# ps-auxw/CLI-P

Hardware: AMD Instinct MI355X
Metric: images/sec ViT-B/32 encode (higher is better)
Workload: dtype bf16

## Files before the change

### cli-p_amd/csrc/encode.hip

```cpp
#include "vit_kernels.hpp"

namespace clipmi {
namespace {

struct Ws {
    unsigned short* patches;
    float* x;
    unsigned short* h;
    unsigned short* big;
    unsigned short* pooled;
    int* rowidx;
    unsigned char* a8;
    float* a_scale;
    unsigned char* a_bs;
    unsigned char* x8;
    unsigned char* x8_bs;
    void* x3;
    float* ln_part;
    float* ln_leaf;
};

size_t carve(const clipmi_tower* t, int B, void* base, size_t cap, Ws* out) {
    Arena ar(base ? base : reinterpret_cast<void*>(256), cap);
    const size_t rows = (size_t)B * t->tokens;
    const int W = t->width;
    Ws w{};
    if (t->kind == 0) w.patches = ar.take<unsigned short>((size_t)B * (t->tokens - 1) * t->patch_k);
    w.x = ar.take<float>(rows * W);
    w.h = ar.take<unsigned short>(rows * W);
    w.big = ar.take<unsigned short>(rows * 4 * W);
    w.pooled = ar.take<unsigned short>((size_t)B * W);
    w.rowidx = ar.take<int>((size_t)B);
    if (t->weight_format == 1) {
        w.a8 = ar.take<unsigned char>(rows * 4 * W);
        w.a_scale = ar.take<float>(rows);
        w.a_bs = ar.take<unsigned char>((rows + 255) / 256 * 256 * (size_t)(4 * W / 32));
    }
    if (t->ln_fold && t->weight_format == 1) {
        w.x8 = ar.take<unsigned char>(rows * W);
        w.x8_bs = ar.take<unsigned char>((rows + 255) / 256 * 256 * (size_t)(W / 32));
        w.ln_part = ar.take<float>(rows * 2 * (W / 256));
    } else if (t->ln_fold) {
        w.x3 = ar.take<unsigned char>(rows * resid_row_bytes(W));
        w.ln_part = ar.take<float>(rows * 2 * (W / 256));
        if (rows <= (size_t)SKINNY_MAX_M) w.ln_leaf = ar.take<float>(rows * 2 * (W / 4));
    }
    if (out) *out = w;
    return ar.off + 256;
}

int check_tower(const clipmi_tower* t, int kind, const char* who) {
    if (!t) return set_err(CLIPMI_EINVAL, "%s: NULL tower", who);
    if (t->abi_version != CLIPMI_ABI_VERSION)
        return set_err(CLIPMI_EINVAL, "%s: tower ABI %d != %d", who, t->abi_version, CLIPMI_ABI_VERSION);
    if (t->kind != kind) return set_err(CLIPMI_EINVAL, "%s: tower kind %d", who, t->kind);
    if (t->width % 128 != 0 || t->heads * 64 != t->width || t->mlp != 4 * t->width || t->embed % 128 != 0 ||
        t->width > 1024 || t->layers < 1)
        return set_err(CLIPMI_EUNSUPPORTED,
                       "%s: width=%d heads=%d mlp=%d embed=%d (need width %% 128 == 0 <= 1024, head dim 64, embed %% 128 == 0)",
                       who, t->width, t->heads, t->mlp, t->embed);
    if (t->weight_format != 0 && t->weight_format != 1)
        return set_err(CLIPMI_EINVAL, "%s: weight_format %d", who, t->weight_format);
    if (t->weight_format == 1 && t->width % 256 != 0)
        return set_err(CLIPMI_EUNSUPPORTED, "%s: fp8 weights need width %% 256 == 0 (width %d)", who, t->width);
    if (t->ln_fold != 0 && (t->ln_fold != 1 || t->width % 256 != 0))
        return set_err(CLIPMI_EINVAL, "%s: ln_fold %d needs width %% 256 == 0 (width %d)", who, t->ln_fold, t->width);
#ifndef CLIPMI_DEV
    if (t->ln_fold != 0 && t->weight_format != 0)
        return set_err(CLIPMI_EUNSUPPORTED, "%s: folded LayerNorms on FP8 weights exist in the development library only", who);
#endif
    if (t->tokens > 80 && kind == 1)
        return set_err(CLIPMI_EUNSUPPORTED, "%s: %d tokens (causal attention covers <= 80)", who, t->tokens);
    return 0;
}

template <typename T>
const T* at(const void* blob, uint64_t off) {
    return reinterpret_cast<const T*>(static_cast<const char*>(blob) + off);
}

int run_layers(const clipmi_tower* t, const void* blob, const Ws& w, int B, int causal, hipStream_t st, GemmProbe* probe) {
    const int W = t->width, L = t->tokens, M = B * L;
    const bool fp8 = t->weight_format == 1;
    auto linear = [&](const unsigned short* A, int K, uint64_t w_off, uint64_t b_off, void* out, int N, int epi) -> int {
        GemmArgs g{};
        g.bias = at<float>(blob, b_off); g.out = out; g.M = M; g.N = N; g.K = K;
        g.A = A; g.W = at<unsigned short>(blob, w_off);
        return launch_gemm_algo(g, epi, 0, st, probe);
    };
#ifdef CLIPMI_DEV
    if (t->ln_fold && fp8) {
        auto lnfold8 = [&](uint64_t w_off, uint64_t s_off, uint64_t cb_off, uint64_t cs_off, void* out, unsigned char* out_bs, int N,
                           int epi) -> int {
            GemmArgs g{};
            g.A = reinterpret_cast<const unsigned short*>(w.x8); g.a_bscale = w.x8_bs;
            g.W = at<unsigned short>(blob, w_off); g.w_scale = at<float>(blob, s_off);
            g.bias = at<float>(blob, cb_off); g.colsum = at<float>(blob, cs_off); g.ln_part_in = w.ln_part;
            g.out = out; g.out_bscale = out_bs; g.M = M; g.N = N; g.K = W;
            return launch_gemm_fp8(g, epi, st);
        };
        auto resid8 = [&](const unsigned char* A8, int K, uint64_t w_off, uint64_t s_off, uint64_t b_off) -> int {
            GemmArgs g{};
            g.A = reinterpret_cast<const unsigned short*>(A8); g.a_bscale = w.a_bs;
            g.W = at<unsigned short>(blob, w_off); g.w_scale = at<float>(blob, s_off); g.bias = at<float>(blob, b_off);
            g.out = w.x; g.x8 = w.x8; g.x8_bs = w.x8_bs; g.ln_part = w.ln_part; g.M = M; g.N = W; g.K = K;
            return launch_gemm_fp8(g, EPI_BIAS_RESID_LN8, st);
        };
        unsigned char* const big8 = reinterpret_cast<unsigned char*>(w.big);
        static const bool fuse_off = dev_knob("CLIPMI_FP8_FUSE", 1) == 0;
        for (int l = 0; l < t->layers; ++l) {
            const uint64_t lb = t->off_layers + (uint64_t)l * t->layer_stride;
            if (int rc = lnfold8(lb + t->lo_qkv_w, lb + t->lo_qkv_s, lb + t->lo_qkv_cb, lb + t->lo_qkv_colsum, w.big, nullptr, 3 * W, EPI_LN_BIAS_BF16)) return rc;
            bool fused = false;
            if (int rc = launch_attention(w.big, w.h, B, L, t->heads, causal, 1, st, fuse_off ? nullptr : w.a8, w.a_bs, &fused)) return rc;
            if (!fused)
                if (int rc = launch_quantize_rows_fp8mx(w.h, w.a8, w.a_bs, M, W, st)) return rc;
            if (int rc = resid8(w.a8, W, lb + t->lo_out_w, lb + t->lo_out_s, lb + t->lo_out_b)) return rc;
            if (!fuse_off) {
                if (int rc = lnfold8(lb + t->lo_fc_w, lb + t->lo_fc_s, lb + t->lo_fc_cb, lb + t->lo_fc_colsum, big8, w.a_bs, 4 * W, EPI_LN_BIAS_QGELU_BF16)) return rc;
                if (int rc = resid8(big8, 4 * W, lb + t->lo_proj_w, lb + t->lo_proj_s, lb + t->lo_proj_b)) return rc;
            } else {
                if (int rc = lnfold8(lb + t->lo_fc_w, lb + t->lo_fc_s, lb + t->lo_fc_cb, lb + t->lo_fc_colsum, w.big, nullptr, 4 * W, EPI_LN_BIAS_QGELU_BF16)) return rc;
                if (int rc = launch_quantize_rows_fp8mx(w.big, w.a8, w.a_bs, M, 4 * W, st)) return rc;
                if (int rc = resid8(w.a8, 4 * W, lb + t->lo_proj_w, lb + t->lo_proj_s, lb + t->lo_proj_b)) return rc;
            }
        }
        return 0;
    }
#endif
    if (t->ln_fold) {
        auto lb_of = [&](int l) { return t->off_layers + (uint64_t)l * t->layer_stride; };
        const bool leaf_mode = w.ln_leaf != nullptr && gemm_resid_writes_leaves(M, W, W) && gemm_resid_writes_leaves(M, W, 4 * W);
        bool leaves = false;
        auto ln_linear = [&](uint64_t w_off, uint64_t cb_off, uint64_t cs_off, int N, int epi) -> int {
            GemmArgs g{};
            g.A = static_cast<const unsigned short*>(w.x3); g.lda_bytes = (unsigned)resid_row_bytes(W);
            g.W = at<unsigned short>(blob, w_off); g.bias = at<float>(blob, cb_off);
            g.colsum = at<float>(blob, cs_off); g.ln_part_in = w.ln_part;
            if (leaves) g.ln_leaf_in = w.ln_leaf;
            g.out = w.big; g.M = M; g.N = N; g.K = W;
            return launch_gemm_algo(g, epi, 0, st, probe);
        };
        auto resid_linear = [&](const unsigned short* A, int K, uint64_t w_off, uint64_t b_off) -> int {
            GemmArgs g{};
            g.A = A; g.W = at<unsigned short>(blob, w_off); g.bias = at<float>(blob, b_off);
            g.M = M; g.N = W; g.K = K;
            g.x3 = w.x3; g.ln_part = w.ln_part; g.tmp_f32 = w.x;
            if (leaf_mode) { g.ln_leaf = w.ln_leaf; leaves = true; }
            return launch_gemm_algo(g, EPI_BIAS_RESID_LN_F32, 0, st, probe);
        };
        for (int l = 0; l < t->layers; ++l) {
            const uint64_t lb = lb_of(l);
            if (int rc = ln_linear(lb + t->lo_qkv_w, lb + t->lo_qkv_cb, lb + t->lo_qkv_colsum, 3 * W, EPI_LN_BIAS_BF16)) return rc;
            hipEvent_t* aev = nullptr;
            if (probe && probe->mode == 2 && probe->n < GemmProbe::MAX) {
                const int pi = probe->begin(GemmProbe::EPI_ATTENTION, 2, st, 0);
                aev = &probe->ev[2 * pi];
            }
            if (int rc = launch_attention(w.big, w.h, B, L, t->heads, causal, 1, st, nullptr, nullptr, nullptr, aev)) return rc;
            if (int rc = resid_linear(w.h, W, lb + t->lo_out_w, lb + t->lo_out_b)) return rc;
            if (int rc = ln_linear(lb + t->lo_fc_w, lb + t->lo_fc_cb, lb + t->lo_fc_colsum, 4 * W, EPI_LN_BIAS_QGELU_BF16)) return rc;
            if (int rc = resid_linear(w.big, 4 * W, lb + t->lo_proj_w, lb + t->lo_proj_b)) return rc;
        }
        return 0;
    }
    if (fp8) {
        auto gemm8 = [&](const unsigned char* A8, const float* a_scale, const unsigned char* a_bs, int K, uint64_t w_off,
                         uint64_t s_off, uint64_t b_off, void* out, unsigned char* out_bs, int N, int epi) -> int {
            GemmArgs g{};
            g.bias = at<float>(blob, b_off); g.out = out; g.M = M; g.N = N; g.K = K;
            g.A = reinterpret_cast<const unsigned short*>(A8);
            g.W = at<unsigned short>(blob, w_off);
            g.a_scale = a_scale; g.a_bscale = a_bs; g.out_bscale = out_bs;
            g.w_scale = at<float>(blob, s_off);
            return launch_gemm_fp8(g, epi, st);
        };
        static const bool fuse_off = dev_knob("CLIPMI_FP8_FUSE", 1) == 0;
        const bool fc_mx = !fuse_off && gemm_fp8_emits_mx(M, 4 * W, W);
        unsigned char* const big8 = reinterpret_cast<unsigned char*>(w.big);
        for (int l = 0; l < t->layers; ++l) {
            const uint64_t lb = t->off_layers + (uint64_t)l * t->layer_stride;
            LnArgs ln{w.x, at<float>(blob, lb + t->lo_ln1_w), at<float>(blob, lb + t->lo_ln1_b), w.h, nullptr, 1, M, W, 1};
            ln.out8 = w.a8; ln.scale8 = w.a_scale;
            if (int rc = launch_layernorm(ln, st)) return rc;
            if (int rc = gemm8(w.a8, w.a_scale, nullptr, W, lb + t->lo_qkv_w, lb + t->lo_qkv_s, lb + t->lo_qkv_b, w.big, nullptr, 3 * W, EPI_BIAS_BF16)) return rc;
            bool fused = false;
            if (int rc = launch_attention(w.big, w.h, B, L, t->heads, causal, 1, st, fuse_off ? nullptr : w.a8, w.a_bs, &fused)) return rc;
            if (!fused)
                if (int rc = launch_quantize_rows_fp8mx(w.h, w.a8, w.a_bs, M, W, st)) return rc;
            if (int rc = gemm8(w.a8, nullptr, w.a_bs, W, lb + t->lo_out_w, lb + t->lo_out_s, lb + t->lo_out_b, w.x, nullptr, W, EPI_BIAS_RESID_F32)) return rc;
            ln.w = at<float>(blob, lb + t->lo_ln2_w); ln.b = at<float>(blob, lb + t->lo_ln2_b);
            if (int rc = launch_layernorm(ln, st)) return rc;
            const unsigned char* h8 = w.a8;
            if (fc_mx) {
                if (int rc = gemm8(w.a8, w.a_scale, nullptr, W, lb + t->lo_fc_w, lb + t->lo_fc_s, lb + t->lo_fc_b, big8, w.a_bs, 4 * W, EPI_BIAS_QGELU_BF16)) return rc;
                h8 = big8;
            } else {
                if (int rc = gemm8(w.a8, w.a_scale, nullptr, W, lb + t->lo_fc_w, lb + t->lo_fc_s, lb + t->lo_fc_b, w.big, nullptr, 4 * W, EPI_BIAS_QGELU_BF16)) return rc;
                if (int rc = launch_quantize_rows_fp8mx(w.big, w.a8, w.a_bs, M, 4 * W, st)) return rc;
            }
            if (int rc = gemm8(h8, nullptr, w.a_bs, 4 * W, lb + t->lo_proj_w, lb + t->lo_proj_s, lb + t->lo_proj_b, w.x, nullptr, W, EPI_BIAS_RESID_F32)) return rc;
        }
        return 0;
    }
    for (int l = 0; l < t->layers; ++l) {
        const uint64_t lb = t->off_layers + (uint64_t)l * t->layer_stride;
        LnArgs ln{w.x, at<float>(blob, lb + t->lo_ln1_w), at<float>(blob, lb + t->lo_ln1_b), w.h, nullptr, 1, M, W, 1};
        if (int rc = launch_layernorm(ln, st)) return rc;
        if (int rc = linear(w.h, W, lb + t->lo_qkv_w, lb + t->lo_qkv_b, w.big, 3 * W, EPI_BIAS_BF16)) return rc;
        if (int rc = launch_attention(w.big, w.h, B, L, t->heads, causal, 1, st)) return rc;
        if (int rc = linear(w.h, W, lb + t->lo_out_w, lb + t->lo_out_b, w.x, W, EPI_BIAS_RESID_F32)) return rc;
        ln.w = at<float>(blob, lb + t->lo_ln2_w); ln.b = at<float>(blob, lb + t->lo_ln2_b);
        if (int rc = launch_layernorm(ln, st)) return rc;
        if (int rc = linear(w.h, W, lb + t->lo_fc_w, lb + t->lo_fc_b, w.big, 4 * W, EPI_BIAS_QGELU_BF16)) return rc;
        if (int rc = linear(w.big, 4 * W, lb + t->lo_proj_w, lb + t->lo_proj_b, w.x, W, EPI_BIAS_RESID_F32)) return rc;
    }
    return 0;
}

int run_head(const clipmi_tower* t, const void* blob, const Ws& w, int B, const int* rowidx, long long row_step,
             float* out, int normalize, hipStream_t st) {
    const bool split = t->ln_fold && t->weight_format == 0;
    LnArgs ln{split ? nullptr : w.x, at<float>(blob, t->off_ln_post_w), at<float>(blob, t->off_ln_post_b), w.pooled, rowidx,
              row_step, B, t->width, 1};
    ln.x3 = w.x3;
    if (int rc = launch_layernorm(ln, st)) return rc;
    GemmArgs g{};
    g.A = w.pooled; g.W = at<unsigned short>(blob, t->off_out_proj); g.bias = nullptr; g.out = out;
    g.M = B; g.N = t->embed; g.K = t->width;
    if (int rc = launch_gemm_algo(g, EPI_F32, 0, st)) return rc;
    if (normalize) return clipmi_l2_normalize_rows(out, B, t->embed, st);
    return 0;
}

}
}

using namespace clipmi;

extern "C" size_t clipmi_encode_image_workspace_bytes(const clipmi_tower* t, int B) {
    if (check_tower(t, 0, "encode_image")) return 0;
    if (B < 1) { set_err(CLIPMI_EINVAL, "encode_image: B=%d", B); return 0; }
    return carve(t, B, nullptr, ~(size_t)0, nullptr);
}

static int encode_image_impl(const clipmi_tower* t, const void* blob_dev, const void* pixels_dev, int pix_dtype,
                             int B, float* out_dev, int normalize, void* ws_dev, size_t ws_bytes, void* stream, GemmProbe* probe) {
    if (int rc = check_tower(t, 0, "encode_image")) return rc;
    if (!blob_dev || !pixels_dev || !out_dev || !ws_dev) return set_err(CLIPMI_EINVAL, "encode_image: NULL pointer");
    if (B < 1) return set_err(CLIPMI_EINVAL, "encode_image: B=%d", B);
    if (pix_dtype != CLIPMI_F32 && pix_dtype != CLIPMI_BF16 && pix_dtype != CLIPMI_U8)
        return set_err(CLIPMI_EINVAL, "encode_image: pix_dtype %d", pix_dtype);
    const int grid = t->res / t->patch, np = grid * grid;
    if (np + 1 != t->tokens || t->patch_k % 64 != 0 || t->patch_k < 3 * t->patch * t->patch)
        return set_err(CLIPMI_EINVAL, "encode_image: inconsistent tower (res %d patch %d tokens %d patch_k %d)", t->res,
                       t->patch, t->tokens, t->patch_k);
    const size_t need = clipmi_encode_image_workspace_bytes(t, B);
    if (ws_bytes < need) return set_err(CLIPMI_EWORKSPACE, "encode_image: workspace %zu < %zu", ws_bytes, need);
    Ws w;
    carve(t, B, ws_dev, ws_bytes, &w);
    hipStream_t st = as_stream(stream);
    const int W = t->width, L = t->tokens;

    PatchArgs pa{pixels_dev, w.patches, pix_dtype, B, t->res, t->patch, grid, np, t->patch_k};
    if (int rc = launch_patchify(pa, st)) return rc;
    GemmArgs g{};
    g.A = w.patches; g.W = at<unsigned short>(blob_dev, t->off_patch_w); g.bias = nullptr; g.out = w.x;
    g.M = B * np; g.N = W; g.K = t->patch_k; g.pos = at<float>(blob_dev, t->off_pos); g.np = np; g.L = L;
    if (int rc = launch_gemm_algo(g, EPI_PATCH_F32, 0, st)) return rc;
    hipLaunchKernelGGL(cls_rows_kernel, dim3((unsigned)(((long long)B * W + 255) / 256)), dim3(256), 0, st, w.x,
                       at<float>(blob_dev, t->off_cls), at<float>(blob_dev, t->off_pos), B, L, W);
    CLIPMI_CHECK_LAUNCH("cls_rows_kernel");
    LnArgs ln{w.x, at<float>(blob_dev, t->off_ln_pre_w), at<float>(blob_dev, t->off_ln_pre_b), w.x, nullptr, 1, B * L, W, 0};
    const bool fold8 = t->ln_fold && t->weight_format == 1;
    if (t->ln_fold && !fold8) { ln.out_x3 = w.x3; ln.out_part = w.ln_part; }
    if (int rc = launch_layernorm(ln, st)) return rc;
#ifdef CLIPMI_DEV
    if (fold8)
        if (int rc = launch_rows_mx_stats(w.x, w.x8, w.x8_bs, w.ln_part, B * L, W, st)) return rc;
#endif
    if (int rc = run_layers(t, blob_dev, w, B, 0, st, probe)) return rc;
    return run_head(t, blob_dev, w, B, nullptr, L, out_dev, normalize, st);
}

extern "C" int clipmi_encode_image(const clipmi_tower* t, const void* blob_dev, const void* pixels_dev, int pix_dtype,
                                   int B, float* out_dev, int normalize, void* ws_dev, size_t ws_bytes, void* stream) {
    return encode_image_impl(t, blob_dev, pixels_dev, pix_dtype, B, out_dev, normalize, ws_dev, ws_bytes, stream, nullptr);
}

extern "C" size_t clipmi_encode_text_workspace_bytes(const clipmi_tower* t, int Q) {
    if (check_tower(t, 1, "encode_text")) return 0;
    if (Q < 1) { set_err(CLIPMI_EINVAL, "encode_text: Q=%d", Q); return 0; }
    return carve(t, Q, nullptr, ~(size_t)0, nullptr);
}

extern "C" int clipmi_encode_text(const clipmi_tower* t, const void* blob_dev, const int32_t* ids_dev, int Q,
                                  float* out_dev, int normalize, void* ws_dev, size_t ws_bytes, void* stream) {
    if (int rc = check_tower(t, 1, "encode_text")) return rc;
    if (!blob_dev || !ids_dev || !out_dev || !ws_dev) return set_err(CLIPMI_EINVAL, "encode_text: NULL pointer");
    if (Q < 1) return set_err(CLIPMI_EINVAL, "encode_text: Q=%d", Q);
    const size_t need = clipmi_encode_text_workspace_bytes(t, Q);
    if (ws_bytes < need) return set_err(CLIPMI_EWORKSPACE, "encode_text: workspace %zu < %zu", ws_bytes, need);
    Ws w;
    carve(t, Q, ws_dev, ws_bytes, &w);
    hipStream_t st = as_stream(stream);
    const int W = t->width, L = t->tokens;
    const long long n4 = (long long)Q * L * (W / 4);
    const bool fold8_ = t->ln_fold && t->weight_format == 1;
    if (t->ln_fold && !fold8_ && W % 256 == 0 && W <= 1024) {
        hipLaunchKernelGGL(text_embed_split_kernel, dim3((unsigned)((Q * L + 3) / 4 + 1)), dim3(256), 0, st, ids_dev,
                           at<float>(blob_dev, t->off_tok_emb), at<float>(blob_dev, t->off_pos), w.x3, w.ln_part, w.rowidx, Q, L, W,
                           t->vocab);
        CLIPMI_CHECK_LAUNCH("text_embed_split_kernel");
        if (int rc = run_layers(t, blob_dev, w, Q, 1, st, nullptr)) return rc;
        return run_head(t, blob_dev, w, Q, w.rowidx, 1, out_dev, normalize, st);
    }
    hipLaunchKernelGGL(text_embed_kernel, dim3((unsigned)((n4 + 255) / 256)), dim3(256), 0, st, w.x, ids_dev,
                       at<float>(blob_dev, t->off_tok_emb), at<float>(blob_dev, t->off_pos), Q, L, W, t->vocab);
    CLIPMI_CHECK_LAUNCH("text_embed_kernel");
    hipLaunchKernelGGL(eot_rows_kernel, dim3((Q + 63) / 64), dim3(64), 0, st, ids_dev, w.rowidx, Q, L);
    CLIPMI_CHECK_LAUNCH("eot_rows_kernel");
#ifdef CLIPMI_DEV
    if (t->ln_fold && t->weight_format == 1) {
        if (int rc = launch_rows_mx_stats(w.x, w.x8, w.x8_bs, w.ln_part, Q * L, W, st)) return rc;
    } else
#endif
    if (t->ln_fold) {
        if (int rc = launch_split_stats(w.x, false, w.x3, w.ln_part, Q * L, W, st)) return rc;
    }
    if (int rc = run_layers(t, blob_dev, w, Q, 1, st, nullptr)) return rc;
    return run_head(t, blob_dev, w, Q, w.rowidx, 1, out_dev, normalize, st);
}

static int encode_probe(const clipmi_tower* t, const void* blob_dev, const void* pixels_dev, int pix_dtype, int B, float* out_dev,
                        void* ws_dev, size_t ws_bytes, void* stream, int probe_epi, int reps, int nmodes, float* ms, int* launches,
                        int* kernel_kind, int* epi_ran) {
    if (!ms || reps < 1) return set_err(CLIPMI_EINVAL, "dbg_encode_image_probe_ms: bad arguments");
    const int k_filter = probe_epi >> 8;
    probe_epi &= 0xff;
    GemmProbe p;
    for (int i = 0; i < 2 * GemmProbe::MAX; ++i)
        if (hipEventCreate(&p.ev[i]) != hipSuccess) return set_err(CLIPMI_EHIP, "hipEventCreate");
    for (int i = 0; i < GemmProbe::MAX; ++i)
        if (hipEventCreate(&p.pre[i]) != hipSuccess) return set_err(CLIPMI_EHIP, "hipEventCreate");
    int rc = 0;
    for (int mode = 0; mode < nmodes && rc == 0; ++mode) {
        double total = 0.0;
        int count = 0;
        for (int r = 0; r < reps && rc == 0; ++r) {
            p.epi = probe_epi; p.n = 0; p.mode = mode;
            rc = encode_image_impl(t, blob_dev, pixels_dev, pix_dtype, B, out_dev, 1, ws_dev, ws_bytes, stream, &p);
            if (rc) break;
            if (hipStreamSynchronize(as_stream(stream)) != hipSuccess) { rc = set_err(CLIPMI_EHIP, "hipStreamSynchronize"); break; }
            for (int i = 0; i < p.n; ++i) {
                if (GemmProbe::base_of(p.epi_of[i]) != probe_epi || (k_filter && p.k_of[i] != k_filter)) continue;
                float v = 0.f;
                if (mode == 0) (void)hipEventElapsedTime(&v, p.ev[2 * i], p.ev[2 * i + 1]);
                else if (mode == 1) (void)hipEventElapsedTime(&v, p.pre[i], p.ev[2 * i + 1]);
                else {
                    if (i == 0 || p.kernel_of[i - 1] != 2 ||
                        (p.epi_of[i - 1] != EPI_BIAS_RESID_LN_F32 && p.epi_of[i - 1] != EPI_LN_BIAS_QGELU_BF16 &&
                         p.epi_of[i - 1] != GemmProbe::EPI_ATTENTION)) continue;
                    (void)hipEventElapsedTime(&v, p.ev[2 * (i - 1) + 1], p.ev[2 * i + 1]);
                }
                total += v;
                ++count;
                if (kernel_kind) *kernel_kind = p.kernel_of[i];
                if (epi_ran) *epi_ran = p.epi_of[i];
            }
        }
        if (rc == 0 && count == 0 && mode == 0) rc = set_err(CLIPMI_EINVAL, "dbg_encode_image_probe_ms: no launch matched epi %d", probe_epi);
        if (rc == 0) { ms[mode] = count ? (float)(total / count) : 0.f; if (launches && mode == 0) *launches = count; }
    }
    for (int i = 0; i < 2 * GemmProbe::MAX; ++i) (void)hipEventDestroy(p.ev[i]);
    for (int i = 0; i < GemmProbe::MAX; ++i) (void)hipEventDestroy(p.pre[i]);
    return rc;
}

extern "C" int clipmi_dbg_encode_image_probe_ms(const clipmi_tower* t, const void* blob_dev, const void* pixels_dev,
                                                int pix_dtype, int B, float* out_dev, void* ws_dev, size_t ws_bytes,
                                                void* stream, int probe_epi, int reps, float* kernel_ms, int* launches) {
    return encode_probe(t, blob_dev, pixels_dev, pix_dtype, B, out_dev, ws_dev, ws_bytes, stream, probe_epi, reps, 1, kernel_ms,
                        launches, nullptr, nullptr);
}

extern "C" int clipmi_dbg_encode_image_probe3_ms(const clipmi_tower* t, const void* blob_dev, const void* pixels_dev,
                                                 int pix_dtype, int B, float* out_dev, void* ws_dev, size_t ws_bytes,
                                                 void* stream, int probe_epi, int reps, float* ms3, int* launches,
                                                 int* kernel_kind, int* epi_ran) {
    return encode_probe(t, blob_dev, pixels_dev, pix_dtype, B, out_dev, ws_dev, ws_bytes, stream, probe_epi, reps, 3, ms3,
                        launches, kernel_kind, epi_ran);
}
```

### cli-p_amd/csrc/vit_kernels.hpp

```cpp
#pragma once
#include "gemm.hpp"

namespace clipmi {

struct PatchArgs {
    const void* pix;
    unsigned short* out;
    int dtype, B, R, P, grid, np, patch_k;
};

static __global__ void __launch_bounds__(256) patchify_kernel(PatchArgs a) {
    const long long total = (long long)a.B * a.np * (a.patch_k / 8);
    const long long i = (long long)blockIdx.x * 256 + threadIdx.x;
    if (i >= total) return;
    const int kc = a.patch_k / 8;
    const int k8 = (int)(i % kc);
    const long long bp = i / kc;
    const int p = (int)(bp % a.np);
    const int b = (int)(bp / a.np);
    const int PP = a.P * a.P;
    const float mean[3] = {0.48145466f, 0.4578275f, 0.40821073f};
    const float stdv[3] = {0.26862954f, 0.26130258f, 0.27577711f};
    float v[8];
    if ((a.P & 7) == 0 && (a.R & 7) == 0) {
        const int k = k8 * 8;
        if (k < 3 * PP) {
            const int c = k / PP, rem = k - c * PP;
            const int py = rem / a.P, px = rem - py * a.P;
            const int y = (p / a.grid) * a.P + py, xx = (p % a.grid) * a.P + px;
            const size_t src = (((size_t)b * 3 + c) * a.R + y) * a.R + xx;
            if (a.dtype == CLIPMI_F32) {
                const f32x4 lo = *reinterpret_cast<const f32x4*>(static_cast<const float*>(a.pix) + src);
                const f32x4 hi = *reinterpret_cast<const f32x4*>(static_cast<const float*>(a.pix) + src + 4);
                v[0] = lo.x; v[1] = lo.y; v[2] = lo.z; v[3] = lo.w; v[4] = hi.x; v[5] = hi.y; v[6] = hi.z; v[7] = hi.w;
            } else if (a.dtype == CLIPMI_BF16) {
                const uint4 raw = *reinterpret_cast<const uint4*>(static_cast<const unsigned short*>(a.pix) + src);
                const unsigned w[4] = {raw.x, raw.y, raw.z, raw.w};
#pragma unroll
                for (int j = 0; j < 4; ++j) {
                    v[2 * j] = __uint_as_float(w[j] << 16);
                    v[2 * j + 1] = __uint_as_float(w[j] & 0xffff0000u);
                }
            } else {
                const uint2 raw = *reinterpret_cast<const uint2*>(static_cast<const unsigned char*>(a.pix) + src);
                const float m = mean[c], s = stdv[c];
#pragma unroll
                for (int j = 0; j < 8; ++j) {
                    const unsigned byte = ((j < 4 ? raw.x : raw.y) >> (8 * (j & 3))) & 0xffu;
                    v[j] = ((float)byte / 255.0f - m) / s;
                }
            }
        } else {
#pragma unroll
            for (int j = 0; j < 8; ++j) v[j] = 0.f;
        }
    } else {
#pragma unroll
    for (int j = 0; j < 8; ++j) {
        const int k = k8 * 8 + j;
        float x = 0.f;
        if (k < 3 * PP) {
            const int c = k / PP, rem = k - c * PP;
            const int py = rem / a.P, px = rem - py * a.P;
            const int y = (p / a.grid) * a.P + py, xx = (p % a.grid) * a.P + px;
            const size_t src = (((size_t)b * 3 + c) * a.R + y) * a.R + xx;
            if (a.dtype == CLIPMI_F32) x = static_cast<const float*>(a.pix)[src];
            else if (a.dtype == CLIPMI_BF16) x = bf16_to_f32(static_cast<const unsigned short*>(a.pix)[src]);
            else x = ((float)static_cast<const unsigned char*>(a.pix)[src] / 255.0f - mean[c]) / stdv[c];
        }
        v[j] = x;
    }
    }
    uint4 o = make_uint4(pack_bf16x2(v[0], v[1]), pack_bf16x2(v[2], v[3]), pack_bf16x2(v[4], v[5]), pack_bf16x2(v[6], v[7]));
    *reinterpret_cast<uint4*>(a.out + ((size_t)bp * a.patch_k + k8 * 8)) = o;
}

static __global__ void __launch_bounds__(256) patchify_strip_u8_kernel(PatchArgs a) {
    extern __shared__ __attribute__((aligned(16))) char smem[];
    const int gy = blockIdx.x % a.grid;
    const int c = (blockIdx.x / a.grid) % 3;
    const int b = blockIdx.x / (3 * a.grid);
    const float mean[3] = {0.48145466f, 0.4578275f, 0.40821073f};
    const float stdv[3] = {0.26862954f, 0.26130258f, 0.27577711f};
    const float m = mean[c], sd = stdv[c];
    const unsigned char* src = static_cast<const unsigned char*>(a.pix) + (((size_t)b * 3 + c) * a.R + (size_t)gy * a.P) * a.R;
    unsigned short* lut = reinterpret_cast<unsigned short*>(smem + a.P * a.R);
    lut[threadIdx.x] = (unsigned short)(pack_bf16x2(((float)threadIdx.x / 255.0f - m) / sd, 0.f) & 0xffffu);
    const int nchunk = (a.P * a.R) >> 4;
    for (int j = threadIdx.x; j < nchunk; j += 256)
        *reinterpret_cast<uint4*>(smem + j * 16) = *reinterpret_cast<const uint4*>(src + (size_t)j * 16);
    __syncthreads();
    const int per_patch = (a.P * a.P) >> 3, per_row = a.P >> 3;
    for (int o = threadIdx.x; o < a.grid * per_patch; o += 256) {
        const int gx = o / per_patch, rem = o - gx * per_patch;
        const int y = rem / per_row, px = (rem - y * per_row) << 3;
        const uint2 raw = *reinterpret_cast<const uint2*>(smem + y * a.R + gx * a.P + px);
        unsigned w4[4];
#pragma unroll
        for (int k = 0; k < 4; ++k) {
            const unsigned word = k < 2 ? raw.x : raw.y;
            const unsigned b0 = (word >> (16 * (k & 1))) & 0xffu, b1 = (word >> (16 * (k & 1) + 8)) & 0xffu;
            w4[k] = (unsigned)lut[b0] | ((unsigned)lut[b1] << 16);
        }
        unsigned short* dst = a.out + ((size_t)b * a.np + gy * a.grid + gx) * a.patch_k + c * a.P * a.P + y * a.P + px;
        *reinterpret_cast<uint4*>(dst) = make_uint4(w4[0], w4[1], w4[2], w4[3]);
    }
}

static __global__ void __launch_bounds__(256) cls_rows_kernel(float* x, const float* cls, const float* pos, int B, int L, int W) {
    const long long i = (long long)blockIdx.x * 256 + threadIdx.x;
    if (i >= (long long)B * W) return;
    const int b = (int)(i / W), c = (int)(i - (long long)b * W);
    x[(size_t)b * L * W + c] = cls[c] + pos[c];
}

static __global__ void __launch_bounds__(256) text_embed_kernel(float* x, const int* ids, const float* tok, const float* pos,
                                                         int Q, int L, int W, int vocab) {
    const long long i = (long long)blockIdx.x * 256 + threadIdx.x;
    const int wc = W / 4;
    if (i >= (long long)Q * L * wc) return;
    const int c4 = (int)(i % wc);
    const long long row = i / wc;
    const int t = (int)(row % L);
    int id = ids[row];
    id = id < 0 ? 0 : (id >= vocab ? vocab - 1 : id);
    const f32x4 e = *reinterpret_cast<const f32x4*>(tok + (size_t)id * W + c4 * 4);
    const f32x4 p = *reinterpret_cast<const f32x4*>(pos + (size_t)t * W + c4 * 4);
    *reinterpret_cast<f32x4*>(x + (size_t)row * W + c4 * 4) = e + p;
}

static __global__ void eot_rows_kernel(const int* ids, int* rowidx, int Q, int L) {
    const int q = blockIdx.x * blockDim.x + threadIdx.x;
    if (q >= Q) return;
    int best = ids[(size_t)q * L], bi = 0;
    for (int t = 1; t < L; ++t) {
        const int v = ids[(size_t)q * L + t];
        if (v > best) { best = v; bi = t; }
    }
    rowidx[q] = q * L + bi;
}

struct LnArgs {
    const float* x;
    const float* w;
    const float* b;
    void* out;
    const int* rowidx;
    long long row_step;
    int M, W, out_bf16;
    unsigned char* out8;
    float* scale8;
    const void* x3;
    void* out_x3;
    float* out_part;
};

static __global__ void __launch_bounds__(256) layernorm_kernel(LnArgs a) {
    const int lane = threadIdx.x & 63;
    const int r = blockIdx.x * 4 + (threadIdx.x >> 6);
    if (r >= a.M) return;
    const long long src_row = a.rowidx ? (long long)a.rowidx[r] : (long long)r * a.row_step;
    const float* p = a.x + src_row * a.W;
    f32x4 v[4];
    float s = 0.f;
#pragma unroll
    for (int i = 0; i < 4; ++i) {
        const int c = i * 256 + lane * 4;
        v[i] = f32x4{0.f, 0.f, 0.f, 0.f};
        if (c < a.W) {
            if (a.x) v[i] = *reinterpret_cast<const f32x4*>(p + c);
            else v[i] = split_join(*reinterpret_cast<const uint2*>(resid_hi(a.x3, (size_t)src_row, a.W) + c),
                                   *reinterpret_cast<const unsigned*>(resid_lo(a.x3, (size_t)src_row, a.W) + c));
        }
        s += v[i].x + v[i].y + v[i].z + v[i].w;
    }
#pragma unroll
    for (int o = 32; o >= 1; o >>= 1) s += __shfl_xor(s, o);
    const float mean = s / (float)a.W;
    float q = 0.f;
#pragma unroll
    for (int i = 0; i < 4; ++i) {
        const int c = i * 256 + lane * 4;
        if (c < a.W) {
            const f32x4 d = v[i] - mean;
            q += d.x * d.x + d.y * d.y + d.z * d.z + d.w * d.w;
        }
    }
#pragma unroll
    for (int o = 32; o >= 1; o >>= 1) q += __shfl_xor(q, o);
    const float rstd = rsqrtf(q / (float)a.W + 1e-5f);
    if (a.out8) {
        float mx = 0.f;
#pragma unroll
        for (int i = 0; i < 4; ++i) {
            const int c = i * 256 + lane * 4;
            if (c < a.W) {
                const f32x4 g = *reinterpret_cast<const f32x4*>(a.w + c);
                const f32x4 bb = *reinterpret_cast<const f32x4*>(a.b + c);
                const f32x4 y = (v[i] - mean) * rstd * g + bb;
                const unsigned lo = pack_bf16x2(y.x, y.y), hi = pack_bf16x2(y.z, y.w);
                v[i] = f32x4{__uint_as_float(lo << 16), __uint_as_float(lo & 0xffff0000u), __uint_as_float(hi << 16),
                             __uint_as_float(hi & 0xffff0000u)};
                mx = fmaxf(fmaxf(mx, fabsf(v[i].x)), fmaxf(fabsf(v[i].y), fmaxf(fabsf(v[i].z), fabsf(v[i].w))));
            }
        }
#pragma unroll
        for (int o = 32; o >= 1; o >>= 1) mx = fmaxf(mx, __shfl_xor(mx, o));
        const float sc = mx > 0.f ? mx / 448.0f : 1.0f;
        const float inv = 1.0f / sc;
#pragma unroll
        for (int i = 0; i < 4; ++i) {
            const int c = i * 256 + lane * 4;
            if (c < a.W) {
                int pk = 0;
                pk = __builtin_amdgcn_cvt_pk_fp8_f32(v[i].x * inv, v[i].y * inv, pk, false);
                pk = __builtin_amdgcn_cvt_pk_fp8_f32(v[i].z * inv, v[i].w * inv, pk, true);
                *reinterpret_cast<unsigned*>(a.out8 + (size_t)r * a.W + c) = (unsigned)pk;
            }
        }
        if (lane == 0) a.scale8[r] = sc;
        return;
    }
    if (a.out_x3) {
        const int nseg = a.W >> 8;
#pragma unroll
        for (int i = 0; i < 4; ++i) {
            if (i < nseg) {
                const int c = i * 256 + lane * 4;
                const f32x4 g = *reinterpret_cast<const f32x4*>(a.w + c);
                const f32x4 bb = *reinterpret_cast<const f32x4*>(a.b + c);
                const f32x4 y = (v[i] - mean) * rstd * g + bb;
                uint2 nh;
                unsigned nl;
                split_make(y, nh, nl);
                *reinterpret_cast<uint2*>(resid_hi(a.out_x3, (size_t)r, a.W) + c) = nh;
                *reinterpret_cast<unsigned*>(resid_lo(a.out_x3, (size_t)r, a.W) + c) = nl;
                const float sa = ln_wave_sum(ln_lane_sum(y));
                const float sq = ln_wave_sum(ln_lane_sumsq(y));
                if (lane == 0) *reinterpret_cast<f32x2*>(a.out_part + ((size_t)r * nseg + i) * 2) = f32x2{sa, sq};
            }
        }
        return;
    }
#pragma unroll
    for (int i = 0; i < 4; ++i) {
        const int c = i * 256 + lane * 4;
        if (c < a.W) {
            const f32x4 g = *reinterpret_cast<const f32x4*>(a.w + c);
            const f32x4 bb = *reinterpret_cast<const f32x4*>(a.b + c);
            const f32x4 y = (v[i] - mean) * rstd * g + bb;
            if (a.out_bf16)
                *reinterpret_cast<uint2*>(static_cast<unsigned short*>(a.out) + (size_t)r * a.W + c) =
                    make_uint2(pack_bf16x2(y.x, y.y), pack_bf16x2(y.z, y.w));
            else
                *reinterpret_cast<f32x4*>(static_cast<float*>(a.out) + (size_t)r * a.W + c) = y;
        }
    }
}

template <bool ADD>
static __global__ void __launch_bounds__(256) split_stats_kernel(const float* __restrict__ x, void* x3, float* __restrict__ part,
                                                                 int M, int W) {
    const int lane = threadIdx.x & 63;
    const int r = blockIdx.x * 4 + (threadIdx.x >> 6);
    if (r >= M) return;
    const int nseg = W >> 8;
    const float* p = x + (size_t)r * W;
    unsigned short* const hrow = resid_hi(x3, (size_t)r, W);
    unsigned char* const lrow = resid_lo(x3, (size_t)r, W);
#pragma unroll
    for (int j = 0; j < 4; ++j) {
        if (j < nseg) {
            const int c = j * 256 + lane * 4;
            f32x4 v = *reinterpret_cast<const f32x4*>(p + c);
            if (ADD) v = v + split_join(*reinterpret_cast<const uint2*>(hrow + c), *reinterpret_cast<const unsigned*>(lrow + c));
            uint2 nh;
            unsigned nl;
            split_make(v, nh, nl);
            *reinterpret_cast<uint2*>(hrow + c) = nh;
            *reinterpret_cast<unsigned*>(lrow + c) = nl;
            const float sa = ln_wave_sum(ln_lane_sum(v));
            const float sq = ln_wave_sum(ln_lane_sumsq(v));
            if (lane == 0) *reinterpret_cast<f32x2*>(part + ((size_t)r * nseg + j) * 2) = f32x2{sa, sq};
        }
    }
}

static __global__ void __launch_bounds__(256) text_embed_split_kernel(const int* __restrict__ ids, const float* __restrict__ tok,
                                                                      const float* __restrict__ pos, void* x3, float* __restrict__ part,
                                                                      int* __restrict__ rowidx, int Q, int L, int W, int vocab) {
    const int M = Q * L, nrb = (M + 3) / 4;
    if ((int)blockIdx.x >= nrb) {
        for (int q = threadIdx.x; q < Q; q += 256) {
            int best = ids[(size_t)q * L], bi = 0;
            for (int t = 1; t < L; ++t) {
                const int v = ids[(size_t)q * L + t];
                if (v > best) { best = v; bi = t; }
            }
            rowidx[q] = q * L + bi;
        }
        return;
    }
    const int lane = threadIdx.x & 63;
    const int r = blockIdx.x * 4 + (threadIdx.x >> 6);
    if (r >= M) return;
    const int nseg = W >> 8, t = r % L;
    int id = ids[r];
    id = id < 0 ? 0 : (id >= vocab ? vocab - 1 : id);
    unsigned short* const hrow = resid_hi(x3, (size_t)r, W);
    unsigned char* const lrow = resid_lo(x3, (size_t)r, W);
#pragma unroll
    for (int j = 0; j < 4; ++j) {
        if (j < nseg) {
            const int c = j * 256 + lane * 4;
            const f32x4 v = *reinterpret_cast<const f32x4*>(tok + (size_t)id * W + c) + *reinterpret_cast<const f32x4*>(pos + (size_t)t * W + c);
            uint2 nh;
            unsigned nl;
            split_make(v, nh, nl);
            *reinterpret_cast<uint2*>(hrow + c) = nh;
            *reinterpret_cast<unsigned*>(lrow + c) = nl;
            const float sa = ln_wave_sum(ln_lane_sum(v));
            const float sq = ln_wave_sum(ln_lane_sumsq(v));
            if (lane == 0) *reinterpret_cast<f32x2*>(part + ((size_t)r * nseg + j) * 2) = f32x2{sa, sq};
        }
    }
}

typedef short s16x4 __attribute__((ext_vector_type(4)));

template <int NT, bool CAUSAL, bool TR>
__global__ void __launch_bounds__(256) attention_kernel(const unsigned short* __restrict__ qkv,
                                                        unsigned short* __restrict__ out, int B, int L, int heads) {
    extern __shared__ __attribute__((aligned(16))) char smem[];
    constexpr int KS = (NT + 1) / 2;
    constexpr int ROWS = KS * 32;
    const int lane = threadIdx.x & 63;
    const int wave = __builtin_amdgcn_readfirstlane(threadIdx.x >> 6);
    const int fr = lane & 15, fg = lane >> 4;
    const int W = heads * 64;
    const long long item = (long long)blockIdx.x * 4 + wave;
    if (item >= (long long)B * heads) return;
    const int b = (int)(item / heads), h = (int)(item - (long long)b * heads);
    const unsigned short* base = qkv + (size_t)b * L * 3 * W + h * 64;
    const size_t rs = (size_t)3 * W;
    char* vt = smem + wave * (ROWS * 128);

#pragma unroll
    for (int i = 0; i < ROWS / 8; ++i) {
        int row = i * 8 + (lane >> 3);
        const int srcrow = row < L ? row : L - 1;
        const uint4 d = *reinterpret_cast<const uint4*>(base + (size_t)srcrow * rs + 2 * W + (lane & 7) * 8);
        *reinterpret_cast<uint4*>(vt + row * 128 + (lane & 7) * 16) = d;
    }

    bf16x8 kf[NT][2], qf[NT][2];
#pragma unroll
    for (int t = 0; t < NT; ++t) {
        int row = t * 16 + fr;
        row = row < L ? row : L - 1;
        const unsigned short* pr = base + (size_t)row * rs + fg * 8;
        qf[t][0] = *reinterpret_cast<const bf16x8*>(pr);
        qf[t][1] = *reinterpret_cast<const bf16x8*>(pr + 32);
        kf[t][0] = *reinterpret_cast<const bf16x8*>(pr + W);
        kf[t][1] = *reinterpret_cast<const bf16x8*>(pr + W + 32);
    }
    f32x4 s[NT][NT];
#pragma unroll
    for (int kt = 0; kt < NT; ++kt)
#pragma unroll
        for (int qt = 0; qt < NT; ++qt) {
            f32x4 a = {0.f, 0.f, 0.f, 0.f};
            a = __builtin_amdgcn_mfma_f32_16x16x32_bf16(kf[kt][0], qf[qt][0], a, 0, 0, 0);
            a = __builtin_amdgcn_mfma_f32_16x16x32_bf16(kf[kt][1], qf[qt][1], a, 0, 0, 0);
            s[kt][qt] = a;
        }

#pragma unroll
    for (int qt = 0; qt < NT; ++qt) {
        const int qi = qt * 16 + fr;
        float mx = -INFINITY;
#pragma unroll
        for (int kt = 0; kt < NT; ++kt)
#pragma unroll
            for (int r = 0; r < 4; ++r) {
                const int ki = kt * 16 + 4 * fg + r;
                float x = s[kt][qt][r] * 0.125f;
                if (ki >= L || (CAUSAL && ki > qi)) x = -INFINITY;
                s[kt][qt][r] = x;
                mx = fmaxf(mx, x);
            }
        mx = fmaxf(mx, __shfl_xor(mx, 16));
        mx = fmaxf(mx, __shfl_xor(mx, 32));
        float sum = 0.f;
#pragma unroll
        for (int kt = 0; kt < NT; ++kt)
#pragma unroll
            for (int r = 0; r < 4; ++r) {
                const float e = __expf(s[kt][qt][r] - mx);
                s[kt][qt][r] = e;
                sum += e;
            }
        sum += __shfl_xor(sum, 16);
        sum += __shfl_xor(sum, 32);
        const float inv = 1.0f / sum;
#pragma unroll
        for (int kt = 0; kt < NT; ++kt) s[kt][qt] *= inv;
    }

    asm volatile("s_waitcnt lgkmcnt(0)" ::: "memory");
    __builtin_amdgcn_wave_barrier();
    f32x4 o[4][NT];
#pragma unroll
    for (int dt = 0; dt < 4; ++dt)
#pragma unroll
        for (int qt = 0; qt < NT; ++qt) o[dt][qt] = f32x4{0.f, 0.f, 0.f, 0.f};
#pragma unroll
// ... 621 lines not shown
```

Measured before the change: 104,500.

## Prune last ViT layer to CLS rows after attention

After: 109,700, median of 6. 1.05x the previous value.

```diff
diff --git a/cli-p_amd/csrc/encode.hip b/cli-p_amd/csrc/encode.hip
--- a/cli-p_amd/csrc/encode.hip
+++ b/cli-p_amd/csrc/encode.hip
@@ -18,6 +18,10 @@
     void* x3;
     float* ln_part;
     float* ln_leaf;
+    void* x3c;
+    float* partc;
+    float* leafc;
+    float* xc;
 };
 
 size_t carve(const clipmi_tower* t, int B, void* base, size_t cap, Ws* out) {
@@ -44,6 +48,15 @@
         w.x3 = ar.take<unsigned char>(rows * resid_row_bytes(W));
         w.ln_part = ar.take<float>(rows * 2 * (W / 256));
         if (rows <= (size_t)SKINNY_MAX_M) w.ln_leaf = ar.take<float>(rows * 2 * (W / 4));
+    }
+    if (t->kind == 0 && t->weight_format == 0) {
+        if (t->ln_fold) {
+            w.x3c = ar.take<unsigned char>((size_t)B * resid_row_bytes(W));
+            w.partc = ar.take<float>((size_t)B * 2 * (W / 256));
+            if (B <= SKINNY_MAX_M) w.leafc = ar.take<float>((size_t)B * 2 * (W / 4));
+        } else {
+            w.xc = ar.take<float>((size_t)B * W);
+        }
     }
     if (out) *out = w;
     return ar.off + 256;
@@ -79,9 +92,26 @@
     return reinterpret_cast<const T*>(static_cast<const char*>(blob) + off);
 }
 
-int run_layers(const clipmi_tower* t, const void* blob, const Ws& w, int B, int causal, hipStream_t st, GemmProbe* probe) {
+bool encode_tail() {
+    static const int mode = (int)dev_knob("CLIPMI_ENCODE_TAIL", 1);
+    return mode != 0;
+}
+
+int launch_gather_rows(const void* src, void* dst, int B, int L, size_t row_bytes, hipStream_t st) {
+    if (row_bytes % 16 != 0) return set_err(CLIPMI_EINVAL, "gather_rows: %zu bytes per row", row_bytes);
+    const int row16 = (int)(row_bytes / 16);
+    hipLaunchKernelGGL(gather_rows_kernel, dim3((unsigned)(((long long)B * row16 + 255) / 256)), dim3(256), 0, st,
+                       static_cast<const uint4*>(src), static_cast<uint4*>(dst), B, L, row16);
+    CLIPMI_CHECK_LAUNCH("gather_rows_kernel");
+    return 0;
+}
+
+int run_layers(const clipmi_tower* t, const void* blob, const Ws& w, int B, int causal, hipStream_t st, GemmProbe* probe,
+               bool* pruned = nullptr) {
     const int W = t->width, L = t->tokens, M = B * L;
     const bool fp8 = t->weight_format == 1;
+    const bool tail = pruned && !causal && !fp8 && (t->ln_fold ? w.x3c != nullptr : w.xc != nullptr) && encode_tail();
+    if (pruned) *pruned = tail;
     auto linear = [&](const unsigned short* A, int K, uint64_t w_off, uint64_t b_off, void* out, int N, int epi) -> int {
         GemmArgs g{};
         g.bias = at<float>(blob, b_off); g.out = out; g.M = M; g.N = N; g.K = K;
@@ -152,6 +182,28 @@
         for (int l = 0; l < t->layers; ++l) {
             const uint64_t lb = lb_of(l);
             if (int rc = ln_linear(lb + t->lo_qkv_w, lb + t->lo_qkv_cb, lb + t->lo_qkv_colsum, 3 * W, EPI_LN_BIAS_BF16)) return rc;
+            if (tail && l == t->layers - 1) {
+                const bool tleaf = w.leafc != nullptr && gemm_resid_writes_leaves(B, W, W) && gemm_resid_writes_leaves(B, W, 4 * W);
+                if (int rc = launch_attention(w.big, w.h, B, L, t->heads, causal, 1, st)) return rc;
+                if (int rc = launch_gather_rows(w.x3, w.x3c, B, L, resid_row_bytes(W), st)) return rc;
+                auto tail_resid = [&](const unsigned short* A, unsigned lda_bytes, int K, uint64_t w_off, uint64_t b_off) -> int {
+                    GemmArgs g{};
+                    g.A = A; g.lda_bytes = lda_bytes; g.W = at<unsigned short>(blob, w_off); g.bias = at<float>(blob, b_off);
+                    g.M = B; g.N = W; g.K = K;
+                    g.x3 = w.x3c; g.ln_part = w.partc; g.tmp_f32 = w.x;
+                    if (tleaf) g.ln_leaf = w.leafc;
+                    return launch_gemm_algo(g, EPI_BIAS_RESID_LN_F32, 0, st, nullptr);
+                };
+                if (int rc = tail_resid(w.h, (unsigned)((size_t)L * W * 2), W, lb + t->lo_out_w, lb + t->lo_out_b)) return rc;
+                GemmArgs g{};
+                g.A = static_cast<const unsigned short*>(w.x3c); g.lda_bytes = (unsigned)resid_row_bytes(W);
+                g.W = at<unsigned short>(blob, lb + t->lo_fc_w); g.bias = at<float>(blob, lb + t->lo_fc_cb);
+                g.colsum = at<float>(blob, lb + t->lo_fc_colsum); g.ln_part_in = w.partc;
+                if (tleaf) g.ln_leaf_in = w.leafc;
+                g.out = w.big; g.M = B; g.N = 4 * W; g.K = W;
+                if (int rc = launch_gemm_algo(g, EPI_LN_BIAS_QGELU_BF16, 0, st, nullptr)) return rc;
+                return tail_resid(w.big, 0u, 4 * W, lb + t->lo_proj_w, lb + t->lo_proj_b);
+            }
             hipEvent_t* aev = nullptr;
             if (probe && probe->mode == 2 && probe->n < GemmProbe::MAX) {
                 const int pi = probe->begin(GemmProbe::EPI_ATTENTION, 2, st, 0);
@@ -209,6 +261,21 @@
         if (int rc = launch_layernorm(ln, st)) return rc;
         if (int rc = linear(w.h, W, lb + t->lo_qkv_w, lb + t->lo_qkv_b, w.big, 3 * W, EPI_BIAS_BF16)) return rc;
         if (int rc = launch_attention(w.big, w.h, B, L, t->heads, causal, 1, st)) return rc;
+        if (tail && l == t->layers - 1) {
+            if (int rc = launch_gather_rows(w.x, w.xc, B, L, (size_t)W * 4, st)) return rc;
+            auto tail_linear = [&](const unsigned short* A, unsigned lda_bytes, int K, uint64_t w_off, uint64_t b_off, void* out, int N,
+                                   int epi) -> int {
+                GemmArgs g{};
+                g.A = A; g.lda_bytes = lda_bytes; g.W = at<unsigned short>(blob, w_off); g.bias = at<float>(blob, b_off);
+                g.out = out; g.M = B; g.N = N; g.K = K;
+                return launch_gemm_algo(g, epi, 0, st, nullptr);
+            };
+            if (int rc = tail_linear(w.h, (unsigned)((size_t)L * W * 2), W, lb + t->lo_out_w, lb + t->lo_out_b, w.xc, W, EPI_BIAS_RESID_F32)) return rc;
+            LnArgs ln2{w.xc, at<float>(blob, lb + t->lo_ln2_w), at<float>(blob, lb + t->lo_ln2_b), w.h, nullptr, 1, B, W, 1};
+            if (int rc = launch_layernorm(ln2, st)) return rc;
+            if (int rc = tail_linear(w.h, 0u, W, lb + t->lo_fc_w, lb + t->lo_fc_b, w.big, 4 * W, EPI_BIAS_QGELU_BF16)) return rc;
+            return tail_linear(w.big, 0u, 4 * W, lb + t->lo_proj_w, lb + t->lo_proj_b, w.xc, W, EPI_BIAS_RESID_F32);
+        }
         if (int rc = linear(w.h, W, lb + t->lo_out_w, lb + t->lo_out_b, w.x, W, EPI_BIAS_RESID_F32)) return rc;
         ln.w = at<float>(blob, lb + t->lo_ln2_w); ln.b = at<float>(blob, lb + t->lo_ln2_b);
         if (int rc = launch_layernorm(ln, st)) return rc;
@@ -279,7 +346,13 @@
     if (fold8)
         if (int rc = launch_rows_mx_stats(w.x, w.x8, w.x8_bs, w.ln_part, B * L, W, st)) return rc;
 #endif
-    if (int rc = run_layers(t, blob_dev, w, B, 0, st, probe)) return rc;
+    bool pruned = false;
+    if (int rc = run_layers(t, blob_dev, w, B, 0, st, probe, &pruned)) return rc;
+    if (pruned) {
+        Ws wc = w;
+        wc.x = w.xc; wc.x3 = w.x3c;
+        return run_head(t, blob_dev, wc, B, nullptr, 1, out_dev, normalize, st);
+    }
     return run_head(t, blob_dev, w, B, nullptr, L, out_dev, normalize, st);
 }
 
diff --git a/cli-p_amd/csrc/vit_kernels.hpp b/cli-p_amd/csrc/vit_kernels.hpp
--- a/cli-p_amd/csrc/vit_kernels.hpp
+++ b/cli-p_amd/csrc/vit_kernels.hpp
@@ -112,6 +112,14 @@
     if (i >= (long long)B * W) return;
     const int b = (int)(i / W), c = (int)(i - (long long)b * W);
     x[(size_t)b * L * W + c] = cls[c] + pos[c];
+}
+
+static __global__ void __launch_bounds__(256) gather_rows_kernel(const uint4* __restrict__ src, uint4* __restrict__ dst, int B,
+                                                                 int row_step, int row16) {
+    const long long i = (long long)blockIdx.x * 256 + threadIdx.x;
+    if (i >= (long long)B * row16) return;
+    const int b = (int)(i / row16), c = (int)(i - (long long)b * row16);
+    dst[(size_t)b * row16 + c] = src[(size_t)b * row_step * row16 + c];
 }
 
 static __global__ void __launch_bounds__(256) text_embed_kernel(float* x, const int* ids, const float* tok, const float* pos,
```
